# miaoyin390/DNN-Compression-Tensor-ADMM

Hardware: AMD Instinct MI355X
Metric: ADMM projection iters/sec (all layers) + per-layer SVD GFLOP/s, ResNet-50 TT ranks (higher is better)
Workload: dtype f32 (Gram, eigen-solve and its filter products accumulate in f64); 1 GPU; resnet50_tt: 34 layers, 20099072 weights, hp table tt_resnet50_hp.HyperParamsDictGeneralRatio3x; tables=1, parallelism=layer-shard x1 (latency-model partition, one scalar all-reduce per step)

## Files before the change

dnn-compression-tensor-admm_amd/csrc/abi_ops.hip:

```cpp
#include "host.h"

using namespace tadmm;

__global__ void square_copy_kernel(const double* __restrict__ in, double* __restrict__ out, int n) {
  const int i = blockIdx.x * blockDim.x + threadIdx.x;
  if (i < n) out[i] = in[i] * in[i];
}

static GemmDesc to_gemm_desc(const tadmm_gemm_desc& s) {
  GemmDesc g;
  memset(&g, 0, sizeof g);
  g.A = s.A; g.B = s.B; g.C = s.C; g.M = s.M; g.N = s.N; g.K = s.K;
  g.a_rs = s.a_rs; g.a_cs = s.a_cs; g.b_rs = s.b_rs; g.b_cs = s.b_cs; g.c_rs = s.c_rs; g.c_cs = s.c_cs;
  g.alpha = s.alpha; g.beta = s.beta; g.bias_n = s.bias_n; g.bias_m = s.bias_m;
  return g;
}

extern "C" {

int tadmm_version(void) { return 100; }

int tadmm_abi_sizes(int* layer_desc_bytes, int* gemm_desc_bytes) {
  if (layer_desc_bytes) *layer_desc_bytes = (int)sizeof(tadmm_layer_desc);
  if (gemm_desc_bytes) *gemm_desc_bytes = (int)sizeof(tadmm_gemm_desc);
// ... 620 lines not shown
  for (int i = 0; i < nprob; ++i) {
    const tadmm_dgemm_tile_prob& q = p[i];
    auto named = [&](int sel, const void* ptr) {
      if (sel < 0) return ptr != nullptr;
      return sel <= 2 && q.ring[0] && q.ring[1] && q.ring[2];
    };
    if (q.M <= 0 || q.N <= 0 || q.K <= 0 || q.M % 32 || q.N % 32 || q.K % 32) return "M, N, K positive multiples of 32";
    if ((q.lda & 1) || (q.ldb & 1) || (q.ldc & 1) || q.lda < q.K || q.ldb < q.K || q.ldc < q.N)
      return "even leading dimensions, lda, ldb >= K, ldc >= N";
    if (q.mode < 0 || q.mode > 3) return "mode 0 .. 3";
    if (!named(q.selC, q.C)) return "C is not named (explicit pointer, or sel 0 .. 2 with a full ring)";
    if (axpby) {
      if (!named(q.selP, q.P) || !q.coef) return "axpby needs P and coef";
    } else {
      if (!named(q.selA, q.A) || !named(q.selB, q.B)) return "A or B is not named";
      if (q.mode >= 1 && !named(q.selP, q.P)) return "modes 1 .. 3 need P";
      if (q.selQ > 2) return "selQ <= 2";
      if (q.selQ >= 0 && !(q.ring[0] && q.ring[1] && q.ring[2])) return "selQ >= 0 needs a full ring";
      if (q.mode == 1 && !q.coef) return "mode 1 needs coef";
      if (q.mode == 3 && !q.theta) return "mode 3 needs theta";
      if (q.mode >= 2 && !q.rowpart) return "modes 2, 3 need rowpart";
    }
  }
  return nullptr;
}

static size_t dgemm_tile_blocks(const tadmm_dgemm_tile_prob& q, int tile_m, int tile_n, int axpby) {
  if (axpby) return (size_t)(((int64_t)q.M * q.ldc + 1023) / 1024);
  return (size_t)((q.M + tile_m - 1) / tile_m) * (size_t)((q.N + tile_n - 1) / tile_n);
}

int tadmm_dgemm_tile_check(int nprob, const tadmm_dgemm_tile_prob* probs, int tile_m, int tile_n, int axpby) {
  return dgemm_tile_refusal(nprob, probs, tile_m, tile_n, axpby) ? TADMM_ERR_INVALID : TADMM_OK;
}

size_t tadmm_dgemm_tile_scratch_bytes(int nprob, const tadmm_dgemm_tile_prob* probs) {
  if (nprob <= 0 || !probs) return 0;
  size_t blocks = 0;
  for (int i = 0; i < nprob; ++i)
    blocks += std::max(dgemm_tile_blocks(probs[i], 32, 32, 0), dgemm_tile_blocks(probs[i], 32, 32, 1));
  return align_up((size_t)nprob * sizeof(DgemmDesc), 256) + align_up(blocks * sizeof(BlockRef), 256);
}

int tadmm_dgemm_tile_f64(tadmm_handle h, int nprob, const tadmm_dgemm_tile_prob* probs, int tile_m, int tile_n, int axpby,
                         void* scratch, size_t scratch_bytes, void* stream_) {
  DeviceGuard device_guard(h);
  if (!h || !scratch) return TADMM_ERR_INVALID;
  if (const char* why = dgemm_tile_refusal(nprob, probs, tile_m, tile_n, axpby))
    CTX_FAIL(h, TADMM_ERR_INVALID, "tadmm_dgemm_tile_f64: %s", why);
  if (scratch_bytes < tadmm_dgemm_tile_scratch_bytes(nprob, probs)) CTX_FAIL(h, TADMM_ERR_WORKSPACE, "dgemm tile scratch too small");
  hipStream_t s = (hipStream_t)stream_;
  std::vector<DgemmDesc> descs((size_t)nprob);
  std::vector<BlockRef> map;
  for (int i = 0; i < nprob; ++i) {
    const tadmm_dgemm_tile_prob& q = probs[i];
    DgemmDesc& g = descs[(size_t)i];
    memset(&g, 0, sizeof g);
    g.A = q.A; g.B = q.B; g.C = q.C; g.P = q.P; g.Q = q.Q;
    g.ring[0] = q.ring[0]; g.ring[1] = q.ring[1]; g.ring[2] = q.ring[2]; g.rot = q.rot;
    g.selA = q.selA; g.selB = q.selB; g.selC = q.selC; g.selP = q.selP; g.selQ = q.selQ;
    g.M = q.M; g.N = q.N; g.K = q.K; g.lda = q.lda; g.ldb = q.ldb; g.ldc = q.ldc;
    g.tiles_m = q.M / 32; g.tiles_n = q.N / 32; g.mode = q.mode;
    g.coef = q.coef; g.theta = q.theta; g.rowpart = q.rowpart; g.gate = q.gate; g.gate_min = q.gate_min;
    const int nb = (int)dgemm_tile_blocks(q, tile_m, tile_n, axpby);
    for (int b = 0; b < nb; ++b) map.push_back(BlockRef{i, b});
  }
  DgemmDesc* gd = (DgemmDesc*)scratch;
  BlockRef* md = (BlockRef*)((char*)scratch + align_up((size_t)nprob * sizeof(DgemmDesc), 256));
  HIP_OK(h, hipMemcpyAsync(gd, descs.data(), descs.size() * sizeof(DgemmDesc), hipMemcpyHostToDevice, s));
  HIP_OK(h, hipMemcpyAsync(md, map.data(), map.size() * sizeof(BlockRef), hipMemcpyHostToDevice, s));
  HIP_OK(h, hipStreamSynchronize(s));
  if (axpby) launch_daxpby(gd, md, (int)map.size(), s);
  else launch_dgemm_nt64(gd, md, (int)map.size(), s, tile_n, tile_m);
  HIP_OK(h, hipStreamSynchronize(s));
  HIP_OK(h, hipGetLastError());
  return TADMM_OK;
}

}
```

dnn-compression-tensor-admm_amd/csrc/filter_host.h:

```cpp
#pragma once
#include <memory>
#include "host.h"

namespace tadmm {

static inline int filter_block_size(int N, int r) {
  const char* e = getenv("TADMM_FILTER");
  if (e && !atoi(e)) return 0;
  int min_n = 192;
  if (const char* m = getenv("TADMM_FILTER_MINN")) min_n = atoi(m);
  if (N < min_n || r < 16) return 0;
  double over = 1.45;
  if (const char* o = getenv("TADMM_FILTER_OVERSAMPLE")) over = atof(o);
  int rp = (int)align_up((size_t)(over * r + 0.999), 32);
  double min_over = 1.15;
  if (const char* o = getenv("TADMM_FILTER_MIN_OVERSAMPLE")) min_over = atof(o);
  if (rp > 256) {
    rp = 256;
    if ((double)rp < min_over * r) return 0;
  }
  if (rp * 100 > 56 * N || rp <= r) return 0;
  return rp;
}

// ... 86 lines not shown
  size_t zero_off = 0, zero_bytes = 0;
  Phase gplanes, stage0_f, p1_f;
  std::vector<Phase> steps_f;
  int fast_stages = -1;
  int last_stages = 0, last_bad = 0;
};

static inline int filter_fast_stages(const FilterGroup& fg) {
  const char* on = getenv("TADMM_FILTER_FAST");
  if (!on || !atoi(on)) return 0;
  if (const char* e = getenv("TADMM_FILTER_FAST_STAGES")) return std::max(0, atoi(e));
  return std::max(0, fg.fast_stages);
}

struct FilterRR { EigDesc desc; int norm_blocks; int ext_blocks; };

template <class DevFn>
static inline void filter_layout(FilterGroup& fg, const std::vector<FilterSpec>& specs, Arena& da, Arena& ar, DevFn dev,
                                 HostImage* img, std::vector<FilterRR>& rr_out) {
  const int nf = (int)specs.size();
  fg.nf = nf;
  rr_out.clear();
  if (nf == 0) return;
  fg.max_degree = 8;
  {
    bool all_comp = true;
    for (const FilterSpec& f : specs) all_comp = all_comp && f.comp_r > 0;
    if (all_comp) fg.max_degree = 16;
    bool all_wide = !all_comp;
    for (const FilterSpec& f : specs) all_wide = all_wide && f.comp_r == 0 && 10 * f.rp >= 14 * f.r;
    if (all_wide) fg.max_degree = 12;
  }
  if (const char* e = getenv("TADMM_FILTER_DEGREE")) fg.max_degree = std::max(2, std::min(16, atoi(e)));
  {
    int tiles64 = 0, rp_max = 0;
    for (const FilterSpec& f : specs) {
      tiles64 += ((f.rp + 63) / 64) * ((f.Npad + filter_tile_n() - 1) / filter_tile_n());
      rp_max = std::max(rp_max, f.rp);
    }
    fg.tile_m = filter_tile_m(tiles64, rp_max);
  }
  const int D = fg.max_degree;
  std::vector<FiltProb> probs(nf);
  std::vector<DgemmDesc> d_stage0(nf), d_p1(nf), d_axpby(nf), d_tfinal(nf), d_hform(nf), d_uform(nf), d_verify(nf),
      d_gramA(nf), d_gramB(nf);
  std::vector<std::vector<DgemmDesc>> d_steps(std::max(0, D - 1), std::vector<DgemmDesc>(nf));
  std::vector<CholDesc> cA(nf), cB(nf);
  std::vector<BlockRef> m_init, m_stage0, m_axpby, m_hform, m_uform, m_verify, m_emit, m_gram, m_solve, m_fast, m_gp;
  std::vector<GPlaneDesc> d_gp(nf);
  std::vector<CompDesc> d_comp;
  std::vector<DgemmDesc> d_cgram;
  std::vector<CholDesc> c_comp;
  std::vector<BlockRef> m_cform, m_cgram, m_cemit, m_csolve;
  fg.ncomp = 0; fg.comp_npad_max = 0;
  const size_t zero_begin = align_up(ar.off, 256);
  std::vector<size_t> xth_off(nf), vh_offs(nf);
  for (int i = 0; i < nf; ++i) {
    const int ldh = (int)align_up(specs[i].rp, 128);
    xth_off[i] = ar.take((size_t)specs[i].rp * ldh * 8);
    vh_offs[i] = ar.take(align_up(specs[i].r, 32) * (size_t)specs[i].rp * 8);
  }
  fg.zero_off = zero_begin;
  fg.zero_bytes = ar.off - zero_begin;
  for (int i = 0; i < nf; ++i) {
    const FilterSpec& sp = specs[i];
    const int rp = sp.rp, Npad = sp.Npad, r32 = (int)align_up(sp.r, 32), ldy = Npad, ldh = (int)align_up(rp, 128);
    const int TNW = filter_tile_n();
    const int TMW = fg.tile_m;
    const int tn = (Npad + TNW - 1) / TNW, tr = (rp + TMW - 1) / TMW;
    size_t ring_off[3];
    for (auto& o : ring_off) o = ar.take((size_t)rp * ldy * 8);
    const size_t st_off = ar.take(sizeof(FiltState));
    const size_t c_off = ar.take((size_t)rp * rp * 8);
    const size_t r_off = ar.take((size_t)rp * rp * 8);
    const size_t w_off = ar.take((size_t)rp * 16 * 8);
    const size_t rq_off = ar.take((size_t)tn * rp * 8);
    const size_t vp_off = ar.take((size_t)tn * r32 * 8);
    const size_t vh_off = vh_offs[i];
    const int gnt = Npad / 16, gks = Npad / 32;
    const int64_t gplane = (int64_t)gnt * gks * 512;
    const size_t gp_off = ar.take((size_t)3 * gplane * 2);
    {
      GPlaneDesc& gd = d_gp[i];
      memset(&gd, 0, sizeof gd);
      gd.Gm = sp.G; gd.ldg = sp.ldg; gd.nt = gnt; gd.ks = gks; gd.out = (uint16_t*)dev(gp_off); gd.plane = gplane;
    }
    const size_t ut_off = ar.take((size_t)r32 * ldy * 8);
    const size_t th_off = ar.take((size_t)r32 * 8);
    const size_t lam_off = ar.take((size_t)rp * 8);
    const size_t ord_off = ar.take((size_t)rp * 4);
    const size_t off_off = ar.take(3 * 8);
    const size_t done_off = ar.take(4);
    const size_t sblk_off = ar.take((size_t)(rp / 16) * 256 * 8);
    FiltState* st = (FiltState*)dev(st_off);
    double* ring[3] = {(double*)dev(ring_off[0]), (double*)dev(ring_off[1]), (double*)dev(ring_off[2])};

    FiltProb& p = probs[i];
    memset(&p, 0, sizeof p);
    p.st = st;
    for (int k = 0; k < 3; ++k) p.ring[k] = ring[k];
    p.N = sp.N; p.Npad = Npad; p.rp = rp; p.r = sp.r; p.r32 = r32; p.ldy = ldy;
    p.rqpart = (const double*)dev(rq_off); p.rq_tiles = tn;
    p.vpart = (const double*)dev(vp_off); p.v_tiles = tn;
    p.lam = (const double*)dev(lam_off); p.order = (const int32_t*)dev(ord_off);
    p.sigma = sp.sigma; p.theta = (double*)dev(th_off); p.UT = (const double*)dev(ut_off);
    p.mode = sp.mode; p.ldo = sp.ldo; p.out_a = sp.out_a; p.out_b = sp.out_b;
    p.skip_slot = sp.skip_slot; p.fb_skip = sp.fb_skip;
    p.G = sp.G; p.ldg = sp.ldg;
    p.H = (const double*)dev(xth_off[i]); p.ldh = ldh;
    fg.npad_max = std::max(fg.npad_max, Npad); fg.rp_max = std::max(fg.rp_max, rp);
    auto base_desc = [&](int M, int N_, int K) {
      DgemmDesc g;
      memset(&g, 0, sizeof g);
      for (int k = 0; k < 3; ++k) g.ring[k] = ring[k];
      g.selA = g.selB = g.selC = g.selP = g.selQ = -1;
      g.M = M; g.N = N_; g.K = K;
      g.tiles_m = M / 32; g.tiles_n = N_ / 32;
      g.Gp = (const uint16_t*)dev(gp_off); g.g_plane = gplane;
      return g;
    };
    const int32_t* w_base = st ? &st->base : nullptr;
    const int32_t* w_res = st ? &st->res : nullptr;
// ... 50 lines not shown
      cB[i] = c;
    }
    {
      DgemmDesc g = base_desc(rp, Npad, Npad);
      g.rot = w_base; g.selA = 0; g.selC = 1; g.B = sp.G;
      g.lda = ldy; g.ldb = sp.ldg; g.ldc = ldy; g.mode = 0; g.gate = w_alive; g.gate_min = 1;
      d_tfinal[i] = g;
      DgemmDesc hgm = base_desc(rp, rp, Npad);
      hgm.rot = w_base; hgm.selA = 0; hgm.selB = 1; hgm.C = (const double*)dev(xth_off[i]);
      hgm.lda = ldy; hgm.ldb = ldy; hgm.ldc = ldh; hgm.mode = 0; hgm.gate = w_alive; hgm.gate_min = 1;
      d_hform[i] = hgm;
    }
    {
      DgemmDesc g = base_desc(r32, Npad, rp);
      g.rot = w_base; g.A = (const double*)dev(vh_off); g.selB = 0; g.C = (const double*)dev(ut_off);
      g.lda = rp; g.ldb = ldy; g.ldc = ldy; g.mode = 0; g.gate = w_alive; g.gate_min = 1;
      d_uform[i] = g;
      DgemmDesc v = base_desc(r32, Npad, Npad);
      v.A = (const double*)dev(ut_off); v.B = sp.G; v.P = (const double*)dev(ut_off);
      v.lda = ldy; v.ldb = sp.ldg; v.ldc = ldy; v.mode = 3; v.theta = (const double*)dev(th_off);
      v.rowpart = (double*)dev(vp_off); v.gate = w_alive; v.gate_min = 1;
      d_verify[i] = v;
    }
    if (sp.comp_r > 0) {
      const int cr = sp.comp_r, ci = fg.ncomp++;
      fg.comp_npad_max = std::max(fg.comp_npad_max, Npad);
      const size_t cimg_off = ar.take((size_t)cr * ldy * 8);
      const size_t cg_off = ar.take((size_t)cr * cr * 8);
      const size_t cr_off = ar.take((size_t)cr * cr * 8);
      const size_t cw_off = ar.take((size_t)cr * 16 * 8);
      const size_t cs_off = ar.take(8);
      CompDesc cd;
      memset(&cd, 0, sizeof cd);
      cd.st = st; cd.G = sp.g_orig; cd.Gc = (double*)sp.G; cd.N = sp.N; cd.Npad = Npad; cd.ldg = sp.ldg;
      cd.cshift = (double*)dev(cs_off);
      cd.UT = (const double*)dev(ut_off); cd.ldy = ldy; cd.k = sp.r;
      cd.Cimg = (double*)dev(cimg_off); cd.r = cr;
      cd.out_a = sp.out_a; cd.ldo = sp.ldo; cd.sigma_layer = sp.sigma_layer;
      d_comp.push_back(cd);
      DgemmDesc g = base_desc(cr, cr, Npad);
      g.A = (const double*)dev(cimg_off); g.B = (const double*)dev(cimg_off); g.C = (const double*)dev(cg_off);
      g.lda = ldy; g.ldb = ldy; g.ldc = cr; g.mode = 0; g.gate = w_alive; g.gate_min = 1;
      d_cgram.push_back(g);
      CholDesc c;
      memset(&c, 0, sizeof c);
      c.C = (const double*)dev(cg_off); c.ldc = cr; c.n = cr;
      c.R = (double*)dev(cr_off); c.ldr = cr; c.Wd = (double*)dev(cw_off);
      for (int k = 0; k < 3; ++k) c.ring[k] = (double*)dev(cimg_off);
      c.rot = nullptr; c.sel = 0; c.ldy = ldy; c.ncols = Npad;
      c.bad = st ? &st->bad : nullptr; c.rot_out = nullptr;
      c.gate = w_alive; c.gate_min = 1;
      c_comp.push_back(c);
      for (int b = 0; b < (cr + 3) / 4; ++b) { m_cform.push_back(BlockRef{ci, b}); m_cemit.push_back(BlockRef{ci, b}); }
      for (int b = 0; b < ((cr + TMW - 1) / TMW) * ((cr + TNW - 1) / TNW); ++b) m_cgram.push_back(BlockRef{ci, b});
      for (int b = 0; b < Npad / kCholStrip; ++b) m_csolve.push_back(BlockRef{ci, b});
    }

    FilterRR rr;
    memset(&rr, 0, sizeof rr);
    EigDesc& e = rr.desc;
    e.XT = (double*)dev(xth_off[i]);
    e.N = rp; e.Npad = rp; e.ld = ldh; e.nb = rp / kJB;
    e.off = (double*)dev(off_off); e.done = (int32_t*)dev(done_off);
    e.lam = (double*)dev(lam_off); e.order = (int32_t*)dev(ord_off); e.sigma = sp.sigma;
    e.r = sp.r; e.mode = 2; e.evec_out = (double*)dev(vh_off); e.sblk = (double*)dev(sblk_off);
    if (eig_mid_direct_on() && eig_mid_direct_size(rp)) e.scratch = (double*)dev(ar.take(eig_mid_scratch_bytes(rp)));
    rr.norm_blocks = (rp + 3) / 4; rr.ext_blocks = (sp.r + 3) / 4;
    rr_out.push_back(rr);
    const int el_blocks = (int)(((size_t)rp * ldy + 1023) / 1024);
    for (int b = 0; b < el_blocks; ++b) { m_init.push_back(BlockRef{i, b}); m_axpby.push_back(BlockRef{i, b}); }
    for (int b = 0; b < tr * tn; ++b) m_stage0.push_back(BlockRef{i, b});
    for (int b = 0; b < (rp / 32) * ((Npad + 63) / 64); ++b) m_fast.push_back(BlockRef{i, b});
    for (int b = 0; b < (gnt * gks + 3) / 4; ++b) m_gp.push_back(BlockRef{i, b});
    for (int b = 0; b < tr * ((rp + TNW - 1) / TNW); ++b) { m_gram.push_back(BlockRef{i, b}); m_hform.push_back(BlockRef{i, b}); }
    for (int b = 0; b < (r32 / 32) * (Npad / 32); ++b) m_uform.push_back(BlockRef{i, b});
    for (int b = 0; b < ((r32 + TMW - 1) / TMW) * tn; ++b) m_verify.push_back(BlockRef{i, b});
    for (int b = 0; b < (sp.r + 3) / 4; ++b) m_emit.push_back(BlockRef{i, b});
    for (int b = 0; b < Npad / kCholStrip; ++b) m_solve.push_back(BlockRef{i, b});
    (void)vh_off;
  }
  if (const char* e = getenv("TADMM_FILTER_XCD"); e && atoi(e)) {
    std::vector<double> wk(nf);
    for (int i = 0; i < nf; ++i) wk[i] = specs[i].Npad;
    xcd_by_problem(m_stage0, wk);
    if (atoi(e) > 1) {
      xcd_by_problem(m_gram, wk);
      xcd_by_problem(m_hform, wk);
      xcd_by_problem(m_verify, wk);
      xcd_by_problem(m_solve, wk);
    }
  }
  {
    std::vector<int> tn_of(nf);
    for (int i = 0; i < nf; ++i) tn_of[i] = (specs[i].Npad + 63) / 64;
    xcd_by_key(m_fast, [&](const BlockRef& b) { return b.prob * 3 + b.local % tn_of[b.prob]; });
  }
  fg.prob_off = da.take(probs.size() * sizeof(FiltProb));
  if (img) img->put(fg.prob_off, probs.data(), probs.size() * sizeof(FiltProb));
  auto place = [&](Phase& ph, const std::vector<DgemmDesc>& d, const std::vector<BlockRef>& m) {
    place_phase(ph, da, img, d.data(), d.size() * sizeof(DgemmDesc), nf, m);
  };
  place(fg.stage0, d_stage0, m_stage0);
  place(fg.p1, d_p1, m_stage0);
  place(fg.stage0_f, d_stage0, m_fast);
  place(fg.p1_f, d_p1, m_fast);
  fg.steps_f.assign(d_steps.size(), Phase());
  for (size_t k = 0; k < d_steps.size(); ++k) place(fg.steps_f[k], d_steps[k], m_fast);
  place_phase(fg.gplanes, da, img, d_gp.data(), d_gp.size() * sizeof(GPlaneDesc), nf, m_gp);
  place(fg.axpby, d_axpby, m_axpby);
  fg.steps.assign(d_steps.size(), Phase());
  for (size_t k = 0; k < d_steps.size(); ++k) place(fg.steps[k], d_steps[k], m_stage0);
  place(fg.gramA, d_gramA, m_gram);
  place(fg.gramB, d_gramB, m_gram);
  place(fg.tfinal, d_tfinal, m_stage0);
  place(fg.hform, d_hform, m_hform);
  place(fg.uform, d_uform, m_uform);
  place(fg.verify, d_verify, m_verify);
  fg.cholA_off = da.take(cA.size() * sizeof(CholDesc));
  fg.cholB_off = da.take(cB.size() * sizeof(CholDesc));
  fg.solve_map_off = da.take(m_solve.size() * sizeof(BlockRef));
  fg.solve_blocks = (int)m_solve.size();
  {
    fg.init.nprob = nf; fg.init.nblocks = (int)m_init.size();
    fg.init.map_off = da.take(m_init.size() * sizeof(BlockRef));
    fg.emit.nprob = nf; fg.emit.nblocks = (int)m_emit.size();
    fg.emit.map_off = da.take(std::max<size_t>(m_emit.size() * sizeof(BlockRef), 16));
  }
  if (fg.ncomp > 0) {
    fg.comp_off = da.take(d_comp.size() * sizeof(CompDesc));
    if (img) img->put(fg.comp_off, d_comp.data(), d_comp.size() * sizeof(CompDesc));
    place_phase(fg.cform, da, img, nullptr, 0, fg.ncomp, m_cform);
    place_phase(fg.cemit, da, img, nullptr, 0, fg.ncomp, m_cemit);
    place_phase(fg.cgram, da, img, d_cgram.data(), d_cgram.size() * sizeof(DgemmDesc), fg.ncomp, m_cgram);
// ... 193 lines not shown
```

dnn-compression-tensor-admm_amd/csrc/host.h:

```cpp
#pragma once
#include "common.h"

#include <algorithm>
#include <atomic>
#include <cstdio>
#include <cstdlib>
#include <cstring>
#include <functional>
#include <string>
#include <vector>

struct tadmm_ctx_s {
  int device = 0;
  std::string err;
};

#define CTX_FAIL(h, code, ...)                                   \
  do {                                                           \
    char _b[512];                                                \
    snprintf(_b, sizeof _b, __VA_ARGS__);                        \
    if (h) (h)->err = _b;                                        \
    return (code);                                               \
  } while (0)

// ... 140 lines not shown
  std::vector<std::vector<BlockRef>> per(np);
  for (const BlockRef& b : m) per[b.prob].push_back(b);
  std::vector<int> order(np);
  for (int i = 0; i < np; ++i) order[i] = i;
  std::stable_sort(order.begin(), order.end(), [&](int a, int b) {
    return weight[a] * per[a].size() > weight[b] * per[b].size();
  });
  std::vector<std::vector<BlockRef>> bin(8);
  double load[8] = {0};
  for (int p : order) {
    int best = 0;
    for (int x = 1; x < 8; ++x) if (load[x] < load[best]) best = x;
    load[best] += weight[p] * per[p].size();
    bin[best].insert(bin[best].end(), per[p].begin(), per[p].end());
  }
  size_t head[8] = {0};
  std::vector<BlockRef> out;
  out.reserve(G);
  for (int i = 0; (int)out.size() < G; ++i) {
    int x = i & 7;
    if (head[x] >= bin[x].size()) {
      int full = -1; size_t left = 0;
      for (int y = 0; y < 8; ++y) if (bin[y].size() - head[y] > left) { left = bin[y].size() - head[y]; full = y; }
      if (full < 0) break;
      x = full;
    }
    out.push_back(bin[x][head[x]++]);
  }
  m.swap(out);
}

template <class KeyFn>
static inline void xcd_by_key(std::vector<BlockRef>& m, KeyFn key) {
  const char* e = getenv("TADMM_XCD_MAP");
  if (e && !atoi(e)) return;
  const int G = (int)m.size();
  if (G < 64) return;
  std::vector<std::vector<BlockRef>> bin(8);
  for (const BlockRef& b : m) bin[(size_t)(key(b) & 7)].push_back(b);
  size_t head[8] = {0};
  std::vector<BlockRef> out;
  out.reserve(G);
  for (int i = 0; (int)out.size() < G; ++i) {
    int x = i & 7;
    if (head[x] >= bin[x].size()) {
      int full = -1; size_t left = 0;
      for (int y = 0; y < 8; ++y) if (bin[y].size() - head[y] > left) { left = bin[y].size() - head[y]; full = y; }
      if (full < 0) break;
      x = full;
    }
    out.push_back(bin[x][head[x]++]);
  }
  m.swap(out);
}

enum class EigTick {
  Pairs,
  SuperPairs,
};
static inline EigTick choose_eig_tick(int ld_max) {
  const char* em = getenv("TADMM_JACOBI_MODE");
  const bool want_pairs = em && atoi(em) == 0;
  return (!want_pairs && jacobi_tick3_fits(ld_max)) ? EigTick::SuperPairs : EigTick::Pairs;
}

static inline bool align_sweeps_on() {
  static const bool on = !(getenv("TADMM_JACOBI_ALIGN") && !atoi(getenv("TADMM_JACOBI_ALIGN")));
  return on;
}

struct PollCtx {
  hipEvent_t ev[2];
  int* host = nullptr;
  size_t stride = 0;
  bool made = false;
  hipError_t create(size_t max_problems) {
    stride = (max_problems + 1 + 15) & ~(size_t)15;
    hipError_t e = hipHostMalloc((void**)&host, 2 * stride * sizeof(int), hipHostMallocDefault);
    for (int i = 0; i < 2 && e == hipSuccess; ++i) e = hipEventCreateWithFlags(&ev[i], hipEventDisableTiming);
    made = e == hipSuccess;
    return e;
  }
  void destroy() {
    if (!made) return;
    for (auto& e : ev) (void)hipEventDestroy(e);
    (void)hipHostFree(host);
    made = false;
  }
};

struct JacobiTiming {
  bool on = false;
  hipEvent_t a{}, b{};
  double tick_ms = 0.0; int tick_launches = 0; double tick_flops = 0.0; double tick_wgs = 0.0;
  double small_ms = 0.0; int small_launches = 0; double small_flops = 0.0;
  const int* small_n = nullptr;
};

struct EigGroup {
  const EigDesc* ed = nullptr;
  int neig = 0;
  const int* players = nullptr;
  int gsteps = 0;
  EigTick kernel = EigTick::Pairs;
  int ld_max = 0;
  size_t tick_lds = 0;
// ... 245 lines not shown
```

dnn-compression-tensor-admm_amd/tadmm/_cabi.py:

```python
from __future__ import annotations

import ctypes as C
import os
import threading

MAX_MODES = 8

KIND_TT_CONV, KIND_TT_LINEAR, KIND_SVD, KIND_TUCKER2 = 0, 1, 2, 3
FLAG_SKIP_ROTATIONS = 1

_LIB_NAME = "libtadmm_hip.so"
_HERE = os.path.dirname(os.path.abspath(__file__))


class TadmmLibraryError(RuntimeError):
    pass


class TadmmError(RuntimeError):
    def __init__(self, status, msg):
        super().__init__(f"tadmm status {status}: {msg}")
        self.status = status


# ... 31 lines not shown
        ("ldx", C.c_int64), ("ldy", C.c_int64), ("win_plane", C.c_int64), ("wout_plane", C.c_int64),
        ("x_hw", C.c_int32), ("y_hw", C.c_int32), ("dtype", C.c_int32), ("tile_tokens", C.c_int32),
    ]


class ConvChainDesc(C.Structure):
    _fields_ = [
        ("X", C.c_void_p), ("Y", C.c_void_p), ("W1", C.c_void_p), ("W2", C.c_void_p), ("W3", C.c_void_p),
        ("bias", C.c_void_p),
        ("w1_plane", C.c_int64), ("w2_plane", C.c_int64), ("w3_plane", C.c_int64),
        ("B", C.c_int32), ("C", C.c_int32), ("R1", C.c_int32), ("R2", C.c_int32), ("Nout", C.c_int32),
        ("H", C.c_int32), ("W", C.c_int32), ("Ho", C.c_int32), ("Wo", C.c_int32), ("kh", C.c_int32), ("kw", C.c_int32),
        ("stride_h", C.c_int32), ("stride_w", C.c_int32), ("pad_h", C.c_int32), ("pad_w", C.c_int32),
        ("dil_h", C.c_int32), ("dil_w", C.c_int32), ("dtype", C.c_int32),
    ]


CHAIN_F32, CHAIN_BF16, CHAIN_F16 = 0, 1, 2
CONV_CHAIN_FWD, CONV_CHAIN_BWD = 0, 1


class OrthDesc(C.Structure):
    _fields_ = [
        ("P", C.c_void_p), ("grad_offset", C.c_int64), ("rows", C.c_int32), ("cols", C.c_int32),
        ("ld", C.c_int64), ("gram_of_rows", C.c_int32), ("reserved", C.c_int32),
    ]


class StiefelDesc(C.Structure):
    _fields_ = [
        ("X", C.c_void_p), ("G", C.c_void_p), ("M", C.c_void_p), ("rows", C.c_int32), ("cols", C.c_int32),
        ("ld", C.c_int64),
    ]


BERTADAM_CHUNK = 4096


class BertAdamDesc(C.Structure):
    _fields_ = [("p", C.c_void_p), ("g", C.c_void_p), ("m", C.c_void_p), ("v", C.c_void_p), ("n", C.c_int64)]


class DgemmTileProb(C.Structure):
    _fields_ = [
        ("A", C.c_void_p), ("B", C.c_void_p), ("C", C.c_void_p), ("P", C.c_void_p), ("Q", C.c_void_p),
        ("ring", C.c_void_p * 3), ("rot", C.c_void_p),
        ("selA", C.c_int32), ("selB", C.c_int32), ("selC", C.c_int32), ("selP", C.c_int32), ("selQ", C.c_int32),
        ("M", C.c_int32), ("N", C.c_int32), ("K", C.c_int32),
        ("lda", C.c_int32), ("ldb", C.c_int32), ("ldc", C.c_int32),
        ("mode", C.c_int32),
        ("coef", C.c_void_p), ("theta", C.c_void_p), ("rowpart", C.c_void_p),
        ("gate", C.c_void_p), ("gate_min", C.c_int32),
    ]


TTM_MAX_D = 4


class TtmDesc(C.Structure):
    _fields_ = [
        ("cores", C.c_void_p * TTM_MAX_D), ("dcores", C.c_void_p * TTM_MAX_D),
        ("order", C.c_void_p * TTM_MAX_D), ("offsets", C.c_void_p * TTM_MAX_D),
        ("index", C.c_void_p), ("dY", C.c_void_p), ("Y", C.c_void_p), ("bad_count", C.c_void_p),
        ("B", C.c_int64), ("d", C.c_int32), ("index_dtype", C.c_int32),
        ("n", C.c_int32 * TTM_MAX_D), ("m", C.c_int32 * TTM_MAX_D), ("r", C.c_int32 * (TTM_MAX_D + 1)),
        ("reserved", C.c_int32),
    ]


class LstmDesc(C.Structure):
    _fields_ = [
        ("Xp", C.c_void_p), ("W", C.c_void_p), ("h0", C.c_void_p), ("c0", C.c_void_p),
        ("Y", C.c_void_p), ("hT", C.c_void_p), ("cT", C.c_void_p), ("G", C.c_void_p), ("C", C.c_void_p),
        ("dY", C.c_void_p), ("dhT", C.c_void_p), ("dcT", C.c_void_p),
        ("dZ", C.c_void_p), ("dh0", C.c_void_p), ("dc0", C.c_void_p),
        ("T", C.c_int64), ("B", C.c_int64), ("H", C.c_int32), ("sigmoid", C.c_int32),
    ]


DISTILL_BASE_NONE, DISTILL_BASE_INDEX, DISTILL_BASE_DENSE = 0, 1, 2
DISTILL_KD_NONE, DISTILL_KD_SOFT_KL, DISTILL_KD_HARD, DISTILL_KD_SOFT_CE = 0, 1, 2, 3


class DistillDesc(C.Structure):
    _fields_ = [
        ("s", C.c_void_p), ("k", C.c_void_p), ("t", C.c_void_p),
        ("s_ld", C.c_int64), ("k_ld", C.c_int64), ("t_ld", C.c_int64),
        ("labels", C.c_void_p), ("dense", C.c_void_p), ("dense_ld", C.c_int64),
        ("workspace", C.c_void_p), ("workspace_bytes", C.c_size_t),
        ("loss_dev", C.c_void_p), ("loss_f32_dev", C.c_void_p), ("counts_dev", C.c_void_p),
        ("grad_s", C.c_void_p), ("grad_k", C.c_void_p),
        ("ignore_index", C.c_int64),
        ("eps", C.c_double), ("alpha", C.c_double), ("tau", C.c_double),
        ("B", C.c_int32), ("C", C.c_int32), ("dtype", C.c_int32),
        ("base_kind", C.c_int32), ("kd_kind", C.c_int32), ("reserved", C.c_int32),
    ]


LAYER_MSE_MAX_PAIRS = 32
LAYER_MSE_ATT, LAYER_MSE_REP = 0, 1


class LayerMsePair(C.Structure):
    _fields_ = [
        ("s", C.c_void_p), ("t", C.c_void_p), ("grad", C.c_void_p),
        ("n", C.c_int64), ("scale", C.c_double), ("thr", C.c_float),
# ... 241 lines not shown
    "tadmm_bertnorm_bwd": (C.c_int, [C.c_void_p, C.POINTER(BertNormDesc), C.c_void_p]),
    "tadmm_prenorm_desc_bytes": (C.c_int, []),
    "tadmm_prenorm_fits": (C.c_int, [C.POINTER(PreNormDesc), C.POINTER(C.c_int)]),
    "tadmm_prenorm_workspace_bytes": (C.c_int, [C.POINTER(PreNormDesc), C.POINTER(C.c_size_t)]),
    "tadmm_prenorm_fwd": (C.c_int, [C.c_void_p, C.POINTER(PreNormDesc), C.c_void_p]),
    "tadmm_prenorm_bwd": (C.c_int, [C.c_void_p, C.POINTER(PreNormDesc), C.c_void_p]),
    "tadmm_bnact_desc_bytes": (C.c_int, []),
    "tadmm_bnact_fits": (C.c_int, [C.POINTER(BnActDesc), C.POINTER(C.c_int64)]),
    "tadmm_bnact_workspace_bytes": (C.c_int, [C.POINTER(BnActDesc), C.POINTER(C.c_size_t)]),
    "tadmm_bnact_plan": (C.c_int, [C.POINTER(BnActDesc), C.POINTER(C.c_int32)]),
    "tadmm_bnact_fwd": (C.c_int, [C.c_void_p, C.POINTER(BnActDesc), C.c_void_p]),
    "tadmm_bnact_bwd": (C.c_int, [C.c_void_p, C.POINTER(BnActDesc), C.c_void_p]),
    "tadmm_densebn_desc_bytes": (C.c_int, []),
    "tadmm_densebn_max_segments": (C.c_int, []),
    "tadmm_densebn_fits": (C.c_int, [C.POINTER(DenseBnDesc), C.POINTER(C.c_int64)]),
    "tadmm_densebn_workspace_bytes": (C.c_int, [C.POINTER(DenseBnDesc), C.POINTER(C.c_size_t)]),
    "tadmm_densebn_plan": (C.c_int, [C.POINTER(DenseBnDesc), C.POINTER(C.c_int32)]),
    "tadmm_densebn_stats": (C.c_int, [C.c_void_p, C.POINTER(DenseBnDesc), C.c_void_p]),
    "tadmm_densebn_fwd": (C.c_int, [C.c_void_p, C.POINTER(DenseBnDesc), C.c_void_p]),
    "tadmm_densebn_bwd": (C.c_int, [C.c_void_p, C.POINTER(DenseBnDesc), C.c_void_p]),
    "tadmm_dwbn_desc_bytes": (C.c_int, []),
    "tadmm_dwbn_fits": (C.c_int, [C.POINTER(DwBnDesc), C.POINTER(C.c_int32)]),
    "tadmm_dwbn_plan": (C.c_int, [C.POINTER(DwBnDesc), C.POINTER(C.c_int32)]),
    "tadmm_dwbn_workspace_bytes": (C.c_int, [C.POINTER(DwBnDesc), C.POINTER(C.c_size_t)]),
    "tadmm_dwbn_fwd": (C.c_int, [C.c_void_p, C.POINTER(DwBnDesc), C.c_void_p]),
    "tadmm_dwbn_bwd": (C.c_int, [C.c_void_p, C.POINTER(DwBnDesc), C.c_void_p]),
    "tadmm_core_conv_desc_bytes": (C.c_int, []),
    "tadmm_core_conv_fwd": (C.c_int, [C.c_void_p, C.POINTER(CoreConvDesc), C.c_void_p]),
    "tadmm_core_conv_dgrad": (C.c_int, [C.c_void_p, C.POINTER(CoreConvDesc), C.c_void_p]),
    "tadmm_core_conv_wgrad_workspace_bytes": (C.c_int, [C.POINTER(CoreConvDesc), C.POINTER(C.c_size_t),
                                                        C.POINTER(C.c_int)]),
    "tadmm_core_conv_wgrad": (C.c_int, [C.c_void_p, C.POINTER(CoreConvDesc), C.c_void_p, C.c_void_p, C.c_size_t,
                                        C.c_void_p]),
    "tadmm_gram_scratch_bytes": (C.c_size_t, [C.c_int, C.c_int]),
    "tadmm_gram_ld": (C.c_int, [C.c_int, C.c_int, C.POINTER(C.c_int), C.POINTER(C.c_int)]),
    "tadmm_gram_f64": (C.c_int, [C.c_void_p, C.c_void_p, C.c_int, C.c_int, C.c_void_p, C.c_int, C.c_void_p,
                                 C.c_size_t, C.c_void_p]),
    "tadmm_eigh_scratch_bytes": (C.c_size_t, [C.c_int]),
    "tadmm_eigh_f64": (C.c_int, [C.c_void_p, C.c_void_p, C.c_int, C.c_void_p, C.c_void_p, C.c_void_p, C.c_size_t,
                                 C.POINTER(C.c_int), C.c_void_p]),
    "tadmm_eigh_partial_f64": (C.c_int, [C.c_void_p, C.c_void_p, C.c_int, C.c_int, C.c_void_p, C.c_void_p, C.c_void_p,
                                         C.c_size_t, C.POINTER(C.c_int), C.c_void_p]),
    "tadmm_dgemm_scratch_bytes": (C.c_size_t, [C.c_int, C.c_int]),
    "tadmm_dgemm3_scratch_bytes": (C.c_size_t, [C.c_int, C.c_int]),
    "tadmm_dgemm3_f64": (C.c_int, [C.c_void_p, C.c_void_p, C.c_void_p, C.c_void_p, C.c_int, C.c_int, C.c_int, C.c_int,
                                   C.c_int, C.c_int, C.c_void_p, C.c_size_t, C.c_void_p]),
    "tadmm_dgemm_f64": (C.c_int, [C.c_void_p, C.c_void_p, C.c_void_p, C.c_void_p, C.c_int, C.c_int, C.c_int, C.c_int,
                                  C.c_int, C.c_int, C.c_int, C.c_void_p, C.c_size_t, C.c_void_p]),
    "tadmm_dgemm_tile_prob_bytes": (C.c_int, []),
    "tadmm_dgemm_tile_check": (C.c_int, [C.c_int, C.POINTER(DgemmTileProb), C.c_int, C.c_int, C.c_int]),
    "tadmm_dgemm_tile_scratch_bytes": (C.c_size_t, [C.c_int, C.POINTER(DgemmTileProb)]),
    "tadmm_dgemm_tile_f64": (C.c_int, [C.c_void_p, C.c_int, C.POINTER(DgemmTileProb), C.c_int, C.c_int, C.c_int,
                                       C.c_void_p, C.c_size_t, C.c_void_p]),
    "tadmm_cholqr_scratch_bytes": (C.c_size_t, [C.c_int, C.c_int]),
    "tadmm_cholqr_f64": (C.c_int, [C.c_void_p, C.c_void_p, C.c_int, C.c_int, C.c_int, C.c_void_p, C.c_size_t,
                                   C.POINTER(C.c_int), C.c_void_p]),
}

_lib = None
_lock = threading.Lock()


def library_path():
    return os.path.join(_HERE, os.path.basename(os.environ.get("TADMM_LIB", _LIB_NAME)))


def load():
    global _lib
    with _lock:
        if _lib is not None:
            return _lib
        import torch
        path = library_path()
        if not os.path.exists(path):
            raise TadmmLibraryError(
                f"{path} not found: build it with `make -C dnn-compression-tensor-admm_amd/csrc` "
                "(or __graft_entry__.build()); there is no CPU fallback")
        try:
            lib = C.CDLL(path)
        except OSError as e:
            raise TadmmLibraryError(f"cannot load {path}: {e}") from e
        missing = []
        for name, (res, args) in ABI.items():
            try:
                fn = getattr(lib, name)
            except AttributeError:
                missing.append(name)
                continue
            fn.restype = res
            fn.argtypes = args
        if missing:
            raise TadmmLibraryError(f"{path} does not export: {', '.join(missing)}")
        a, b = C.c_int(), C.c_int()
        lib.tadmm_abi_sizes(C.byref(a), C.byref(b))
        if (a.value, b.value) != (C.sizeof(LayerDesc), C.sizeof(GemmDesc)):
            raise TadmmLibraryError(f"{path}: struct layout mismatch (library {a.value}/{b.value} bytes, "
                                    f"binding {C.sizeof(LayerDesc)}/{C.sizeof(GemmDesc)})")
        if lib.tadmm_chain_desc_bytes() != C.sizeof(ChainDesc):
            raise TadmmLibraryError(f"{path}: tadmm_chain_desc layout mismatch (library {lib.tadmm_chain_desc_bytes()} "
                                    f"bytes, binding {C.sizeof(ChainDesc)})")
        if lib.tadmm_conv_chain_desc_bytes() != C.sizeof(ConvChainDesc):
            raise TadmmLibraryError(f"{path}: tadmm_conv_chain_desc layout mismatch")
        if lib.tadmm_orth_desc_bytes() != C.sizeof(OrthDesc):
            raise TadmmLibraryError(f"{path}: tadmm_orth_desc layout mismatch")
        if lib.tadmm_stiefel_desc_bytes() != C.sizeof(StiefelDesc):
            raise TadmmLibraryError(f"{path}: tadmm_stiefel_desc layout mismatch")
# ... 111 lines not shown
```

dnn-compression-tensor-admm_amd/tadmm/ops.py:

```python
from __future__ import annotations

import collections
import ctypes as C
import functools
import struct
import weakref
from typing import List, Optional, Sequence

import numpy as np
import torch

from . import _cabi
from ._cabi import (FLAG_SKIP_ROTATIONS, KIND_SVD, KIND_TT_CONV, KIND_TT_LINEAR, KIND_TUCKER2, GemmDesc, Handle,
                    LayerDesc, StiefelDesc, TadmmError, make_layer_desc)


def _handle(device) -> Handle:
    return Handle.get(device.index if device.index is not None else torch.cuda.current_device())


def _stream(device) -> int:
    return torch.cuda.current_stream(device).cuda_stream


# ... 874 lines not shown
        h.check(h.lib.tadmm_eigh_f64(h.ptr, G.data_ptr(), N, *tail))
    else:
        h.check(h.lib.tadmm_eigh_partial_f64(h.ptr, G.data_ptr(), N, int(r), *tail))
    return ev, vec, int(info.value)


def eigh(G: torch.Tensor):
    return _eigh(G, None)


def eigh_partial(G: torch.Tensor, r: int):
    return _eigh(G, r)


def dgemm(a: torch.Tensor, b: torch.Tensor, b_transposed: bool = True) -> torch.Tensor:
    assert a.dtype == torch.float64 and b.dtype == torch.float64 and a.is_cuda and b.is_cuda
    a, b = a.contiguous(), b.contiguous()
    M, K = a.shape
    N = b.shape[0] if b_transposed else b.shape[1]
    out = torch.empty(M, N, dtype=torch.float64, device=a.device)
    h = _handle(a.device)
    scratch = _scratch(h.lib.tadmm_dgemm_scratch_bytes(M, N), a.device)
    h.check(h.lib.tadmm_dgemm_f64(h.ptr, a.data_ptr(), b.data_ptr(), out.data_ptr(), M, N, K, a.stride(0), b.stride(0),
                                  N, int(b_transposed), scratch.data_ptr(), scratch.numel(), _stream(a.device)))
    return out


def dgemm_tile_probs(probs):
    from ._cabi import DgemmTileProb
    arr = (DgemmTileProb * len(probs))()
    ptr = lambda t: None if t is None else t.data_ptr()
    for q, p in zip(arr, probs):
        ring = p.get("ring")
        for name in ("A", "B", "C", "P", "Q", "rot", "coef", "theta", "rowpart", "gate"):
            setattr(q, name, ptr(p.get(name)))
        if ring is not None:
            q.ring[0], q.ring[1], q.ring[2] = (t.data_ptr() for t in ring)
        for name in ("selA", "selB", "selC", "selP", "selQ"):
            setattr(q, name, int(p.get(name, -1)))
        q.M, q.N, q.K, q.mode, q.gate_min = int(p["M"]), int(p["N"]), int(p["K"]), int(p.get("mode", 0)), int(p.get("gate_min", 0))
        for ld, name, sel in (("lda", "A", "selA"), ("ldb", "B", "selB"), ("ldc", "C", "selC")):
            t = p.get(name) if p.get(sel, -1) < 0 else ring[0]
            setattr(q, ld, int(p[ld]) if ld in p else (0 if t is None else t.stride(0)))
    return arr


def dgemm_tile(probs, tile_m: int, tile_n: int, axpby: bool = False, device=None) -> None:
    device = torch.device("cuda", torch.cuda.current_device()) if device is None else device
    arr = dgemm_tile_probs(probs)
    h = _handle(device)
    scratch = _scratch(max(256, h.lib.tadmm_dgemm_tile_scratch_bytes(len(probs), arr)), device)
    h.check(h.lib.tadmm_dgemm_tile_f64(h.ptr, len(probs), arr, tile_m, tile_n, int(axpby), scratch.data_ptr(),
                                       scratch.numel(), _stream(device)))


def dgemm3(a: torch.Tensor, g: torch.Tensor, repeats: int = 1) -> torch.Tensor:
    assert a.dtype == torch.float64 and g.dtype == torch.float64 and a.is_cuda and g.is_cuda
    assert a.is_contiguous() and g.is_contiguous() and g.shape[0] == g.shape[1] == a.shape[1]
    M, N = a.shape
    h = _handle(a.device)
    out = torch.empty(M, N, dtype=torch.float64, device=a.device)
    scratch = _scratch(h.lib.tadmm_dgemm3_scratch_bytes(M, N), a.device)
    h.check(h.lib.tadmm_dgemm3_f64(h.ptr, a.data_ptr(), g.data_ptr(), out.data_ptr(), M, N, N, N, N, repeats,
                                   scratch.data_ptr(), scratch.numel(), _stream(a.device)))
    return out


def cholqr_(yt: torch.Tensor) -> bool:
    assert yt.dtype == torch.float64 and yt.is_cuda and yt.is_contiguous()
    n, ncols = yt.shape
    h = _handle(yt.device)
    scratch = _scratch(h.lib.tadmm_cholqr_scratch_bytes(n, ncols), yt.device)
    bad = C.c_int(0)
    h.check(h.lib.tadmm_cholqr_f64(h.ptr, yt.data_ptr(), n, ncols, yt.stride(0), scratch.data_ptr(), scratch.numel(),
                                   C.byref(bad), _stream(yt.device)))
    return bad.value == 0


STIEFEL_LDS_BYTES = 160 * 1024
STIEFEL_PIVOT_FLOOR = 4e-14
STIEFEL_SECOND_PASS = 1e4


def _align16(v: int) -> int:
    return (v + 15) & ~15


def stiefel_lds_bytes(n: int, p: int) -> int:
    pitch = p | 1
    return 3 * _align16(n * pitch * 4) + 2 * _align16(p * pitch * 8) + 2 * _align16(p * 8)


def stiefel_fits(n: int, p: int) -> bool:
    return 1 <= p <= n and p <= 128 and stiefel_lds_bytes(n, p) <= STIEFEL_LDS_BYTES


def stiefel_desc(x: torch.Tensor, g: Optional[torch.Tensor] = None, m: Optional[torch.Tensor] = None) -> StiefelDesc:
    if x.dim() != 2:
        raise TadmmError(-1, f"a Stiefel factor is a matrix (got shape {tuple(x.shape)})")
    n, p = int(x.shape[0]), int(x.shape[1])
    if p < 1 or n < p:
        raise TadmmError(-1, f"a Stiefel factor is n x p with n >= p >= 1 (got {n} x {p})")
    ld = int(x.stride(0)) if n > 1 else max(int(x.stride(0)), p)
    for what, t in (("factor", x), ("gradient", g), ("momentum buffer", m)):
        if t is None:
            continue
# ... 1533 lines not shown
```

include/tadmm.h:

```cpp
#ifndef TADMM_H_
#define TADMM_H_

#include <stddef.h>
#include <stdint.h>

#ifdef __cplusplus
extern "C" {
#endif

#define TADMM_MAX_MODES 8

typedef enum {
  TADMM_OK = 0,
  TADMM_ERR_INVALID = -1,
  TADMM_ERR_WORKSPACE = -2,
  TADMM_ERR_HIP = -3,
  TADMM_ERR_NOCONVERGE = -4,
  TADMM_ERR_UNSUPPORTED = -5
} tadmm_status;

typedef enum {
  TADMM_KIND_TT_CONV = 0,
  TADMM_KIND_TT_LINEAR = 1,
  TADMM_KIND_SVD = 2,
// ... 454 lines not shown
  tadmm_layer_mse_pair pairs[TADMM_LAYER_MSE_MAX_PAIRS];
  void* workspace; size_t workspace_bytes;
  double* terms_dev;
  double* loss_dev;
  float* loss_f32_dev;
  int32_t npairs;
  int32_t dtype;
} tadmm_layer_mse_desc;
int tadmm_layer_mse_desc_bytes(void);
int tadmm_layer_mse_max_pairs(void);
int tadmm_layer_mse_geometry(int* chunk_elems, int* max_blocks);
int tadmm_layer_mse_workspace_bytes(const tadmm_layer_mse_desc* d, size_t* bytes);
int tadmm_layer_mse(tadmm_handle h, const tadmm_layer_mse_desc* d, void* stream);

size_t tadmm_gram_scratch_bytes(int m, int n);
int tadmm_gram_ld(int m, int n, int* Npad, int* ld);
int tadmm_gram_f64(tadmm_handle h, const float* A, int m, int n, double* G, int ldg,
                   void* partial_dev, size_t partial_bytes, void* stream);

size_t tadmm_eigh_scratch_bytes(int N);
int tadmm_eigh_f64(tadmm_handle h, const double* G, int N, double* evals_out, double* evecs_out,
                   void* scratch_dev, size_t scratch_bytes, int* sweeps_out, void* stream);
int tadmm_eigh_partial_f64(tadmm_handle h, const double* G, int N, int r, double* evals_out, double* evecs_out,
                           void* scratch_dev, size_t scratch_bytes, int* route_out, void* stream);

size_t tadmm_dgemm_scratch_bytes(int M, int N);
int tadmm_dgemm_f64(tadmm_handle h, const double* A, const double* B, double* C, int M, int N, int K, int lda, int ldb,
                    int ldc, int b_transposed, void* scratch, size_t scratch_bytes, void* stream);
size_t tadmm_dgemm3_scratch_bytes(int M, int N);
int tadmm_dgemm3_f64(tadmm_handle h, const double* A, const double* G, double* C, int M, int N, int lda, int ldg, int ldc,
                     int repeats, void* scratch, size_t scratch_bytes, void* stream);
size_t tadmm_cholqr_scratch_bytes(int n, int ncols);
int tadmm_cholqr_f64(tadmm_handle h, double* YT, int n, int ncols, int ldy, void* scratch, size_t scratch_bytes,
                     int* bad_out_host, void* stream);
typedef struct {
  const double* A; const double* B; double* C;
  const double* P; const double* Q;
  double* ring[3];
  const int32_t* rot;
  int32_t selA, selB, selC, selP, selQ;
  int32_t M, N, K;
  int32_t lda, ldb, ldc;
  int32_t mode;
  const double* coef;
  const double* theta;
  double* rowpart;
  const int32_t* gate; int32_t gate_min;
} tadmm_dgemm_tile_prob;
int tadmm_dgemm_tile_prob_bytes(void);
int tadmm_dgemm_tile_check(int nprob, const tadmm_dgemm_tile_prob* probs, int tile_m, int tile_n, int axpby);
size_t tadmm_dgemm_tile_scratch_bytes(int nprob, const tadmm_dgemm_tile_prob* probs);
int tadmm_dgemm_tile_f64(tadmm_handle h, int nprob, const tadmm_dgemm_tile_prob* probs, int tile_m, int tile_n, int axpby,
                         void* scratch, size_t scratch_bytes, void* stream);

#ifdef __cplusplus
}
#endif
#endif
```

Before: 177.7 iters/s.

## Reorder grouped-GEMM tile dispatch into XCD-aware serpentine bands for L2 reuse

Adds a tile-map builder that assigns the tiles of each grouped DGEMM problem to the eight XCD round-robin queues in serpentine row bands. For each problem it picks the band height that minimizes the distinct A/B panel bytes each XCD touches, then orders problems by K, longest first. The builder falls back to the plain order if its estimated traffic is no lower. It is applied to the filter stage0, gram, verify and companion-gram launches and to the generic tile DGEMM path, with the aim of improving per-XCD L2 hit rates. It adds host-side map construction cost and a new ABI query function.

```diff
diff --git a/dnn-compression-tensor-admm_amd/csrc/abi_ops.hip b/dnn-compression-tensor-admm_amd/csrc/abi_ops.hip
--- a/dnn-compression-tensor-admm_amd/csrc/abi_ops.hip
+++ b/dnn-compression-tensor-admm_amd/csrc/abi_ops.hip
@@ -696,6 +696,7 @@
   hipStream_t s = (hipStream_t)stream_;
   std::vector<DgemmDesc> descs((size_t)nprob);
   std::vector<BlockRef> map;
+  std::vector<TileProb> tiles;
   for (int i = 0; i < nprob; ++i) {
     const tadmm_dgemm_tile_prob& q = probs[i];
     DgemmDesc& g = descs[(size_t)i];
@@ -707,8 +708,10 @@
     g.tiles_m = q.M / 32; g.tiles_n = q.N / 32; g.mode = q.mode;
     g.coef = q.coef; g.theta = q.theta; g.rowpart = q.rowpart; g.gate = q.gate; g.gate_min = q.gate_min;
     const int nb = (int)dgemm_tile_blocks(q, tile_m, tile_n, axpby);
-    for (int b = 0; b < nb; ++b) map.push_back(BlockRef{i, b});
-  }
+    if (axpby) for (int b = 0; b < nb; ++b) map.push_back(BlockRef{i, b});
+    else tiles.push_back(TileProb{q.M, q.N, q.K, tile_m, tile_n});
+  }
+  if (!axpby) map = tile_map_build(tiles);
   DgemmDesc* gd = (DgemmDesc*)scratch;
   BlockRef* md = (BlockRef*)((char*)scratch + align_up((size_t)nprob * sizeof(DgemmDesc), 256));
   HIP_OK(h, hipMemcpyAsync(gd, descs.data(), descs.size() * sizeof(DgemmDesc), hipMemcpyHostToDevice, s));
@@ -721,4 +724,23 @@
   return TADMM_OK;
 }
 
-}
+int64_t tadmm_tile_map(int nprob, const tadmm_tile_map_prob* probs, int32_t* map_out, int64_t capacity, double* cost_out) {
+  if (nprob <= 0 || nprob > 4096 || !probs) return TADMM_ERR_INVALID;
+  std::vector<TileProb> t((size_t)nprob);
+  int64_t blocks = 0;
+  for (int i = 0; i < nprob; ++i) {
+    const tadmm_tile_map_prob& q = probs[i];
+    if (q.M <= 0 || q.N <= 0 || q.K <= 0 || q.tile_m <= 0 || q.tile_n <= 0) return TADMM_ERR_INVALID;
+    t[(size_t)i] = TileProb{q.M, q.N, q.K, q.tile_m, q.tile_n};
+    blocks += (int64_t)tile_rows(t[(size_t)i]) * tile_cols(t[(size_t)i]);
+    if (blocks > (1 << 24)) return TADMM_ERR_INVALID;
+  }
+  if (!map_out && !cost_out) return blocks;
+  if (map_out && capacity < blocks) return TADMM_ERR_WORKSPACE;
+  const std::vector<BlockRef> m = tile_map_build(t);
+  if (map_out) memcpy(map_out, m.data(), m.size() * sizeof(BlockRef));
+  if (cost_out) { cost_out[0] = tile_map_cost(m, t); cost_out[1] = tile_map_cost(tile_map_plain(t), t); }
+  return blocks;
+}
+
+}
diff --git a/dnn-compression-tensor-admm_amd/csrc/filter_host.h b/dnn-compression-tensor-admm_amd/csrc/filter_host.h
--- a/dnn-compression-tensor-admm_amd/csrc/filter_host.h
+++ b/dnn-compression-tensor-admm_amd/csrc/filter_host.h
@@ -162,6 +162,7 @@
   std::vector<DgemmDesc> d_cgram;
   std::vector<CholDesc> c_comp;
   std::vector<BlockRef> m_cform, m_cgram, m_cemit, m_csolve;
+  std::vector<TileProb> t_stage0, t_gram, t_verify, t_cgram;
   fg.ncomp = 0; fg.comp_npad_max = 0;
   const size_t zero_begin = align_up(ar.off, 256);
   std::vector<size_t> xth_off(nf), vh_offs(nf);
@@ -177,7 +178,7 @@
     const int rp = sp.rp, Npad = sp.Npad, r32 = (int)align_up(sp.r, 32), ldy = Npad, ldh = (int)align_up(rp, 128);
     const int TNW = filter_tile_n();
     const int TMW = fg.tile_m;
-    const int tn = (Npad + TNW - 1) / TNW, tr = (rp + TMW - 1) / TMW;
+    const int tn = (Npad + TNW - 1) / TNW;
     size_t ring_off[3];
     for (auto& o : ring_off) o = ar.take((size_t)rp * ldy * 8);
     const size_t st_off = ar.take(sizeof(FiltState));
@@ -334,7 +335,7 @@
       c.gate = w_alive; c.gate_min = 1;
       c_comp.push_back(c);
       for (int b = 0; b < (cr + 3) / 4; ++b) { m_cform.push_back(BlockRef{ci, b}); m_cemit.push_back(BlockRef{ci, b}); }
-      for (int b = 0; b < ((cr + TMW - 1) / TMW) * ((cr + TNW - 1) / TNW); ++b) m_cgram.push_back(BlockRef{ci, b});
+      t_cgram.push_back(TileProb{cr, cr, Npad, TMW, TNW});
       for (int b = 0; b < Npad / kCholStrip; ++b) m_csolve.push_back(BlockRef{ci, b});
     }
 
@@ -351,16 +352,23 @@
     rr_out.push_back(rr);
     const int el_blocks = (int)(((size_t)rp * ldy + 1023) / 1024);
     for (int b = 0; b < el_blocks; ++b) { m_init.push_back(BlockRef{i, b}); m_axpby.push_back(BlockRef{i, b}); }
-    for (int b = 0; b < tr * tn; ++b) m_stage0.push_back(BlockRef{i, b});
+    t_stage0.push_back(TileProb{rp, Npad, Npad, TMW, TNW});
     for (int b = 0; b < (rp / 32) * ((Npad + 63) / 64); ++b) m_fast.push_back(BlockRef{i, b});
     for (int b = 0; b < (gnt * gks + 3) / 4; ++b) m_gp.push_back(BlockRef{i, b});
-    for (int b = 0; b < tr * ((rp + TNW - 1) / TNW); ++b) { m_gram.push_back(BlockRef{i, b}); m_hform.push_back(BlockRef{i, b}); }
+    t_gram.push_back(TileProb{rp, rp, Npad, TMW, TNW});
     for (int b = 0; b < (r32 / 32) * (Npad / 32); ++b) m_uform.push_back(BlockRef{i, b});
-    for (int b = 0; b < ((r32 + TMW - 1) / TMW) * tn; ++b) m_verify.push_back(BlockRef{i, b});
+    t_verify.push_back(TileProb{r32, Npad, Npad, TMW, TNW});
     for (int b = 0; b < (sp.r + 3) / 4; ++b) m_emit.push_back(BlockRef{i, b});
     for (int b = 0; b < Npad / kCholStrip; ++b) m_solve.push_back(BlockRef{i, b});
     (void)vh_off;
   }
+  const bool by_problem = getenv("TADMM_FILTER_XCD") && atoi(getenv("TADMM_FILTER_XCD"));
+  auto tile_map = [&](const std::vector<TileProb>& t) { return by_problem ? tile_map_plain(t) : tile_map_build(t); };
+  m_stage0 = tile_map(t_stage0);
+  m_gram = tile_map(t_gram);
+  m_hform = m_gram;
+  m_verify = tile_map(t_verify);
+  m_cgram = tile_map(t_cgram);
   if (const char* e = getenv("TADMM_FILTER_XCD"); e && atoi(e)) {
     std::vector<double> wk(nf);
     for (int i = 0; i < nf; ++i) wk[i] = specs[i].Npad;
diff --git a/dnn-compression-tensor-admm_amd/csrc/host.h b/dnn-compression-tensor-admm_amd/csrc/host.h
--- a/dnn-compression-tensor-admm_amd/csrc/host.h
+++ b/dnn-compression-tensor-admm_amd/csrc/host.h
@@ -216,6 +216,97 @@
     out.push_back(bin[x][head[x]++]);
   }
   m.swap(out);
+}
+
+struct TileProb { int M, N, K, TM, TN; };
+static inline int tile_rows(const TileProb& q) { return (q.M + q.TM - 1) / q.TM; }
+static inline int tile_cols(const TileProb& q) { return (q.N + q.TN - 1) / q.TN; }
+
+static inline int tile_map_mode() {
+  const char* e = getenv("TADMM_XCD_MAP");
+  if (e && !atoi(e)) return 0;
+  const char* b = getenv("TADMM_TILE_MAP");
+  return b ? std::max(0, std::min(2, atoi(b))) : 1;
+}
+
+static inline std::vector<BlockRef> tile_map_plain(const std::vector<TileProb>& probs) {
+  std::vector<BlockRef> m;
+  for (int p = 0; p < (int)probs.size(); ++p)
+    for (int b = 0; b < tile_rows(probs[p]) * tile_cols(probs[p]); ++b) m.push_back(BlockRef{p, b});
+  return m;
+}
+
+static inline double tile_map_cost(const std::vector<BlockRef>& map, const std::vector<TileProb>& probs) {
+  std::vector<int> off(probs.size() + 1, 0);
+  for (size_t p = 0; p < probs.size(); ++p) off[p + 1] = off[p] + tile_rows(probs[p]) + tile_cols(probs[p]);
+  std::vector<char> seen((size_t)8 * off.back(), 0);
+  double bytes = 0;
+  for (size_t i = 0; i < map.size(); ++i) {
+    const TileProb& q = probs[map[i].prob];
+    const int tn = tile_cols(q), tr = tile_rows(q), r = map[i].local / tn, c = map[i].local - r * tn;
+    char* s = seen.data() + (i & 7) * (size_t)off.back() + off[map[i].prob];
+    if (!s[r]) { s[r] = 1; bytes += 8.0 * q.TM * q.K; }
+    if (!s[tr + c]) { s[tr + c] = 1; bytes += 8.0 * q.TN * q.K; }
+  }
+  return bytes;
+}
+
+static inline std::vector<int> tile_band_order(int tr, int tn, int h) {
+  std::vector<int> l;
+  l.reserve((size_t)tr * tn);
+  const int nb = (tr + h - 1) / h;
+  for (int b = 0; b < nb; ++b) {
+    const int r0 = b * tr / nb, r1 = (b + 1) * tr / nb;
+    for (int k = 0; k < tn; ++k) {
+      const int c = (b & 1) ? tn - 1 - k : k;
+      for (int r = r0; r < r1; ++r) l.push_back(r * tn + c);
+    }
+  }
+  return l;
+}
+
+static inline std::vector<BlockRef> tile_map_build(const std::vector<TileProb>& probs) {
+  const int mode = tile_map_mode();
+  std::vector<BlockRef> plain = tile_map_plain(probs);
+  if (mode == 0) return plain;
+  const int np = (int)probs.size();
+  std::vector<std::vector<BlockRef>> run((size_t)np * 8);
+  int fill = 0;
+  for (int p = 0; p < np; ++p) {
+    const TileProb& q = probs[p];
+    const int tr = tile_rows(q), tn = tile_cols(q), n = tr * tn;
+    int cnt[8];
+    for (int x = 0; x < 8; ++x) cnt[x] = n / 8;
+    for (int k = 0; k < n % 8; ++k) ++cnt[(fill + k) & 7];
+    fill = (fill + n) & 7;
+    std::vector<int> best;
+    double best_cost = 0;
+    for (int h = (mode == 2 ? tr : 1); h <= tr; ++h) {
+      std::vector<int> l = tile_band_order(tr, tn, h);
+      double cost = 0;
+      for (int x = 0, i = 0; x < 8; i += cnt[x++]) {
+        std::vector<char> seen((size_t)tr + tn, 0);
+        for (int k = i; k < i + cnt[x]; ++k) {
+          const int r = l[k] / tn, c = l[k] - r * tn;
+          if (!seen[r]) { seen[r] = 1; cost += q.TM; }
+          if (!seen[tr + c]) { seen[tr + c] = 1; cost += q.TN; }
+        }
+      }
+      if (best.empty() || cost <= best_cost) { best.swap(l); best_cost = cost; }
+    }
+    for (int x = 0, i = 0; x < 8; i += cnt[x++])
+      for (int k = i; k < i + cnt[x]; ++k) run[(size_t)p * 8 + x].push_back(BlockRef{p, best[k]});
+  }
+  std::vector<int> order(np);
+  for (int p = 0; p < np; ++p) order[p] = p;
+  if (const char* e = getenv("TADMM_TILE_MAP_LONGEST"); !(e && !atoi(e)))
+    std::stable_sort(order.begin(), order.end(), [&](int a, int b) { return probs[a].K > probs[b].K; });
+  std::vector<BlockRef> queue[8];
+  for (int x = 0; x < 8; ++x)
+    for (int p : order) queue[x].insert(queue[x].end(), run[(size_t)p * 8 + x].begin(), run[(size_t)p * 8 + x].end());
+  std::vector<BlockRef> out(plain.size());
+  for (size_t i = 0; i < out.size(); ++i) out[i] = queue[i & 7][i >> 3];
+  return tile_map_cost(out, probs) <= tile_map_cost(plain, probs) ? out : plain;
 }
 
 enum class EigTick {
diff --git a/dnn-compression-tensor-admm_amd/tadmm/_cabi.py b/dnn-compression-tensor-admm_amd/tadmm/_cabi.py
--- a/dnn-compression-tensor-admm_amd/tadmm/_cabi.py
+++ b/dnn-compression-tensor-admm_amd/tadmm/_cabi.py
@@ -107,6 +107,10 @@
         ("coef", C.c_void_p), ("theta", C.c_void_p), ("rowpart", C.c_void_p),
         ("gate", C.c_void_p), ("gate_min", C.c_int32),
     ]
+
+
+class TileMapProb(C.Structure):
+    _fields_ = [("M", C.c_int32), ("N", C.c_int32), ("K", C.c_int32), ("tile_m", C.c_int32), ("tile_n", C.c_int32)]
 
 
 TTM_MAX_D = 4
@@ -454,6 +458,8 @@
     "tadmm_dgemm_tile_scratch_bytes": (C.c_size_t, [C.c_int, C.POINTER(DgemmTileProb)]),
     "tadmm_dgemm_tile_f64": (C.c_int, [C.c_void_p, C.c_int, C.POINTER(DgemmTileProb), C.c_int, C.c_int, C.c_int,
                                        C.c_void_p, C.c_size_t, C.c_void_p]),
+    "tadmm_tile_map": (C.c_int64, [C.c_int, C.POINTER(TileMapProb), C.POINTER(C.c_int32), C.c_int64,
+                                   C.POINTER(C.c_double)]),
     "tadmm_cholqr_scratch_bytes": (C.c_size_t, [C.c_int, C.c_int]),
     "tadmm_cholqr_f64": (C.c_int, [C.c_void_p, C.c_void_p, C.c_int, C.c_int, C.c_int, C.c_void_p, C.c_size_t,
                                    C.POINTER(C.c_int), C.c_void_p]),
diff --git a/dnn-compression-tensor-admm_amd/tadmm/ops.py b/dnn-compression-tensor-admm_amd/tadmm/ops.py
--- a/dnn-compression-tensor-admm_amd/tadmm/ops.py
+++ b/dnn-compression-tensor-admm_amd/tadmm/ops.py
@@ -950,6 +950,21 @@
     scratch = _scratch(max(256, h.lib.tadmm_dgemm_tile_scratch_bytes(len(probs), arr)), device)
     h.check(h.lib.tadmm_dgemm_tile_f64(h.ptr, len(probs), arr, tile_m, tile_n, int(axpby), scratch.data_ptr(),
                                        scratch.numel(), _stream(device)))
+
+
+def tile_map(probs):
+    import ctypes as C
+    from . import _cabi
+    lib = _cabi.load()
+    arr = (_cabi.TileMapProb * len(probs))(*[_cabi.TileMapProb(*map(int, p)) for p in probs])
+    n = lib.tadmm_tile_map(len(probs), arr, None, 0, None)
+    if n < 0:
+        raise ValueError(f"tadmm_tile_map refuses {probs!r}: status {n}")
+    out = (C.c_int32 * (2 * n))()
+    cost = (C.c_double * 2)()
+    got = lib.tadmm_tile_map(len(probs), arr, out, n, cost)
+    assert got == n, (got, n)
+    return [(out[2 * i], out[2 * i + 1]) for i in range(n)], float(cost[0]), float(cost[1])
 
 
 def dgemm3(a: torch.Tensor, g: torch.Tensor, repeats: int = 1) -> torch.Tensor:
diff --git a/include/tadmm.h b/include/tadmm.h
--- a/include/tadmm.h
+++ b/include/tadmm.h
@@ -530,6 +530,8 @@
 size_t tadmm_dgemm_tile_scratch_bytes(int nprob, const tadmm_dgemm_tile_prob* probs);
 int tadmm_dgemm_tile_f64(tadmm_handle h, int nprob, const tadmm_dgemm_tile_prob* probs, int tile_m, int tile_n, int axpby,
                          void* scratch, size_t scratch_bytes, void* stream);
+typedef struct { int32_t M, N, K, tile_m, tile_n; } tadmm_tile_map_prob;
+int64_t tadmm_tile_map(int nprob, const tadmm_tile_map_prob* probs, int32_t* map_out, int64_t capacity, double* cost_out);
 
 #ifdef __cplusplus
 }
```

After: 182.6 iters/s (median of 6 runs). +2.8%, better.
